# mobiusml/hqq

Measured on NVIDIA H100. Metric: llama3_8b_4bit_gs64_decode_tokens_per_s, higher is better.
Workload: dtype f16

## Files before the change

hqq_b200/csrc/linear_small.cu:

```cuda
#include <string.h>
#include <type_traits>

#include "linear_internal.cuh"

namespace hqq {


constexpr int kMaxProb = 4;

struct SKProb {
  const uint8_t* Wq;
  const void* scale;
  const void* zero;
  const void* bias;
  void* y;
  uint32_t* ytag;
  int N;
  int step;
  int tile0;
};

struct SKArgs {
  SKProb p[kMaxProb];
  int nprob;
  const void* x;
  int M, K;
  int Gk;
  int KB;
  int total_tiles;
  int xop;
  int yop;
  const void* x2;
  const void* xw;
  void* h_out;
  float eps;
  int tp, rank;
  uint32_t* peer_data[8];
  const uint32_t* red_data;
  const uint32_t* xtag;
  const uint32_t* x2tag;
  const int* step_ctr;
  int x_index, x_per_step;
};

#ifdef HQQ_EMU
#define HQQ_ST_RELAXED_SYS(p, v) (*reinterpret_cast<volatile uint32_t*>(p) = (v))
#else
#define HQQ_ST_RELAXED_SYS(p, v) asm volatile("st.relaxed.sys.global.u32 [%0], %1;" ::"l"(p), "r"(v) : "memory")
#endif

template <typename T> struct MT16;
template <> struct MT16<__half> {
  static constexpr uint32_t ONE2 = 0x3C003C00u;
  __device__ __forceinline__ static void mma(float (&d)[4], uint32_t a0, uint32_t a1, uint32_t a2, uint32_t a3, uint32_t b0, uint32_t b1) {
#ifndef HQQ_EMU
    asm volatile("mma.sync.aligned.m16n8k16.row.col.f32.f16.f16.f32 {%0,%1,%2,%3}, {%4,%5,%6,%7}, {%8,%9}, {%0,%1,%2,%3};"
                 : "+f"(d[0]), "+f"(d[1]), "+f"(d[2]), "+f"(d[3])
                 : "r"(a0), "r"(a1), "r"(a2), "r"(a3), "r"(b0), "r"(b1));
#else
    ::emu::mma_m16n8k16<__half>(d, a0, a1, a2, a3, b0, b1, false);
#endif
  }
  __device__ __forceinline__ static void mma0(float (&d)[4], uint32_t a0, uint32_t a1, uint32_t a2, uint32_t a3, uint32_t b0, uint32_t b1) {
#ifndef HQQ_EMU
    asm volatile("mma.sync.aligned.m16n8k16.row.col.f32.f16.f16.f32 {%0,%1,%2,%3}, {%4,%5,%6,%7}, {%8,%9}, {%10,%10,%10,%10};"
                 : "=f"(d[0]), "=f"(d[1]), "=f"(d[2]), "=f"(d[3])
                 : "r"(a0), "r"(a1), "r"(a2), "r"(a3), "r"(b0), "r"(b1), "f"(0.0f));
#else
    ::emu::mma_m16n8k16<__half>(d, a0, a1, a2, a3, b0, b1, true);
#endif
  }
  __device__ __forceinline__ static float ld(const void* p, long long i) { return __half2float(reinterpret_cast<const __half*>(p)[i]); }
  __device__ __forceinline__ static __half cvt(float v, const void* bias, int n) {
    __half o = __float2half_rn(v);
    if (bias) o = __hadd(o, reinterpret_cast<const __half*>(bias)[n]);
    return o;
  }
  __device__ __forceinline__ static void st(void* p, long long i, float v, const void* bias, int n) { reinterpret_cast<__half*>(p)[i] = cvt(v, bias, n); }
};
template <> struct MT16<__nv_bfloat16> {
  static constexpr uint32_t ONE2 = 0x3F803F80u;
  __device__ __forceinline__ static void mma(float (&d)[4], uint32_t a0, uint32_t a1, uint32_t a2, uint32_t a3, uint32_t b0, uint32_t b1) {
#ifndef HQQ_EMU
    asm volatile("mma.sync.aligned.m16n8k16.row.col.f32.bf16.bf16.f32 {%0,%1,%2,%3}, {%4,%5,%6,%7}, {%8,%9}, {%0,%1,%2,%3};"
                 : "+f"(d[0]), "+f"(d[1]), "+f"(d[2]), "+f"(d[3])
                 : "r"(a0), "r"(a1), "r"(a2), "r"(a3), "r"(b0), "r"(b1));
#else
    ::emu::mma_m16n8k16<__nv_bfloat16>(d, a0, a1, a2, a3, b0, b1, false);
#endif
  }
  __device__ __forceinline__ static void mma0(float (&d)[4], uint32_t a0, uint32_t a1, uint32_t a2, uint32_t a3, uint32_t b0, uint32_t b1) {
#ifndef HQQ_EMU
    asm volatile("mma.sync.aligned.m16n8k16.row.col.f32.bf16.bf16.f32 {%0,%1,%2,%3}, {%4,%5,%6,%7}, {%8,%9}, {%10,%10,%10,%10};"
                 : "=f"(d[0]), "=f"(d[1]), "=f"(d[2]), "=f"(d[3])
                 : "r"(a0), "r"(a1), "r"(a2), "r"(a3), "r"(b0), "r"(b1), "f"(0.0f));
#else
    ::emu::mma_m16n8k16<__nv_bfloat16>(d, a0, a1, a2, a3, b0, b1, true);
#endif
  }
  __device__ __forceinline__ static float ld(const void* p, long long i) { return __bfloat162float(reinterpret_cast<const __nv_bfloat16*>(p)[i]); }
  __device__ __forceinline__ static __nv_bfloat16 cvt(float v, const void* bias, int n) {
    __nv_bfloat16 o = __float2bfloat16_rn(v);
    if (bias) o = __hadd(o, reinterpret_cast<const __nv_bfloat16*>(bias)[n]);
    return o;
  }
  __device__ __forceinline__ static void st(void* p, long long i, float v, const void* bias, int n) { reinterpret_cast<__nv_bfloat16*>(p)[i] = cvt(v, bias, n); }
};

template <int LUT>
__device__ __forceinline__ uint32_t lop3(uint32_t a, uint32_t b, uint32_t c) {
#ifdef HQQ_EMU
  return ::emu::lop3(a, b, c, (uint32_t)LUT);
#else
  uint32_t r;
  asm("lop3.b32 %0, %1, %2, %3, %4;" : "=r"(r) : "r"(a), "r"(b), "r"(c), "n"(LUT));
  return r;
#endif
}
__device__ __forceinline__ uint32_t and_or(uint32_t a, uint32_t b, uint32_t c) { return lop3<0xEA>(a, b, c); }

template <typename T, int NBITS> struct Lanes;

template <int NBITS>
struct Lanes<__half, NBITS> {
  static constexpr uint32_t OR = 0x64006400u;
  uint32_t mask_a, mask_b;
  float invV_a, invV_b, offV_a, offV_b;
  __device__ __forceinline__ void init(int sh_a, int sh_b) {
    const uint32_t m = (1u << NBITS) - 1u;
    mask_a = (m << sh_a) * 0x00010001u;
    mask_b = (m << sh_b) * 0x00010001u;
    invV_a = exp2f(-(float)sh_a); invV_b = exp2f(-(float)sh_b);
    offV_a = 1024.0f * invV_a;    offV_b = 1024.0f * invV_b;
  }
  __device__ __forceinline__ void extract(uint32_t w, uint32_t& a0, uint32_t& a1, uint32_t& a2, uint32_t& a3) const {
    const uint32_t wp = prmt(w, 0u, 0x3120u);
    const uint32_t wh = wp >> 8;
    a0 = and_or(wp, mask_a, OR);
    a1 = and_or(wp, mask_b, OR);
    a2 = and_or(wh, mask_a, OR);
    a3 = and_or(wh, mask_b, OR);
  }
  __device__ __forceinline__ void extract_np(uint32_t w, uint32_t& a0, uint32_t& a1, uint32_t& a2, uint32_t& a3) const {
    const uint32_t wh = w >> 8;
    a0 = and_or(w, mask_a, OR);
    a1 = and_or(w, mask_b, OR);
    a2 = and_or(wh, mask_a, OR);
    a3 = and_or(wh, mask_b, OR);
  }
};

template <int NBITS>
struct Lanes<__nv_bfloat16, NBITS> {
  int sh_a, sh_b;
  float invV_a, invV_b, offV_a, offV_b;
  __device__ __forceinline__ void init(int sa, int sb) {
    sh_a = sa; sh_b = sb;
    invV_a = invV_b = 1.0f;
    offV_a = offV_b = 128.0f;
  }
  __device__ __forceinline__ void extract(uint32_t w, uint32_t& a0, uint32_t& a1, uint32_t& a2, uint32_t& a3) const {
    constexpr uint32_t M = ((1u << NBITS) - 1u) * 0x00010001u;
    const uint32_t wp = prmt(w, 0u, 0x3120u);
    a0 = and_or(wp >> sh_a, M, 0x43004300u);
    a1 = and_or(wp >> sh_b, M, 0x43004300u);
    a2 = and_or(wp >> (sh_a + 8), M, 0x43004300u);
    a3 = and_or(wp >> (sh_b + 8), M, 0x43004300u);
  }
  __device__ __forceinline__ void extract_np(uint32_t w, uint32_t& a0, uint32_t& a1, uint32_t& a2, uint32_t& a3) const {
    constexpr uint32_t M = ((1u << NBITS) - 1u) * 0x00010001u;
    a0 = and_or(w >> sh_a, M, 0x43004300u);
    a1 = and_or(w >> sh_b, M, 0x43004300u);
    a2 = and_or(w >> (sh_a + 8), M, 0x43004300u);
    a3 = and_or(w >> (sh_b + 8), M, 0x43004300u);
  }
};

template <>
struct Lanes<__half, 8> {
  static constexpr uint32_t HB = 0x64646464u;
  float invV_a, invV_b, offV_a, offV_b;
  __device__ __forceinline__ void init(int, int) { invV_a = invV_b = 1.0f; offV_a = offV_b = 1024.0f; }
  __device__ __forceinline__ void extract2(uint32_t wa, uint32_t wb, uint32_t& a0, uint32_t& a1, uint32_t& a2, uint32_t& a3) const {
    a0 = prmt(wa, HB, 0x4140u);
    a2 = prmt(wa, HB, 0x4342u);
    a1 = prmt(wb, HB, 0x4140u);
    a3 = prmt(wb, HB, 0x4342u);
  }
  __device__ __forceinline__ void extract2_np(uint32_t wa, uint32_t wb, uint32_t& a0, uint32_t& a1, uint32_t& a2, uint32_t& a3) const {
    a0 = prmt(wa, HB, 0x4240u);
    a2 = prmt(wa, HB, 0x4341u);
    a1 = prmt(wb, HB, 0x4240u);
    a3 = prmt(wb, HB, 0x4341u);
  }
};

__device__ __forceinline__ void cp_async16(void* smem, const void* g) {
#ifdef HQQ_EMU
  ::emu::cp_async(smem, g, 16);
#else
  const uint32_t s = (uint32_t)__cvta_generic_to_shared(smem);
  asm volatile("cp.async.cg.shared.global [%0], [%1], 16;" ::"r"(s), "l"(g) : "memory");
#endif
}
#ifdef HQQ_EMU
__device__ __forceinline__ void cp_async_commit() { ::emu::cp_async_commit(); }
template <int N> __device__ __forceinline__ void cp_async_wait() { ::emu::cp_async_wait(N); }
#else
__device__ __forceinline__ void cp_async_commit() { asm volatile("cp.async.commit_group;" ::: "memory"); }
template <int N>
__device__ __forceinline__ void cp_async_wait() { asm volatile("cp.async.wait_group %0;" ::"n"(N) : "memory"); }
#endif

template <typename T> __device__ __forceinline__ T from_f32_t(float v);
template <> __device__ __forceinline__ __half from_f32_t<__half>(float v) { return __float2half_rn(v); }
template <> __device__ __forceinline__ __nv_bfloat16 from_f32_t<__nv_bfloat16>(float v) { return __float2bfloat16_rn(v); }

template <typename T, int NBITS, int GS, int MT>
struct SKCfg {
  static constexpr int F = 8 / NBITS;
  static constexpr int P = 16 / F;
  static constexpr int MPG = GS / 16;
  static constexpr int GPB = 256 / GS;
  static constexpr int NWV = (F == 1) ? 8 : 4;
  static constexpr int ST = (F == 1) ? 2 : 4;
  static constexpr int W_BYTES = ST * NWV * 256 * 16;
  static constexpr int P_BYTES = 2 * 8 * MT * 128 * 4;
  static constexpr int SMEM = W_BYTES + P_BYTES;
  static constexpr int MIN_CTAS = (SMEM <= 110 * 1024 && MT <= 2) ? 2 : 1;
};

template <typename T, int NBITS, int GS, int MT>
__global__ void __launch_bounds__(256, SKCfg<T, NBITS, GS, MT>::MIN_CTAS) linear_small_kernel(const __grid_constant__ SKArgs a) {
  using C = SKCfg<T, NBITS, GS, MT>;
  constexpr int F = C::F, P = C::P, MPG = C::MPG, GPB = C::GPB, NWV = C::NWV, ST = C::ST;
  using MM = MT16<T>;
  extern __shared__ __align__(16) uint8_t smem[];
  uint4* wring = reinterpret_cast<uint4*>(smem);
  float* part_s = reinterpret_cast<float*>(smem + C::W_BYTES);

  const int tid = threadIdx.x, warp = tid >> 5, lane = tid & 31;
  const int r = lane >> 2, c = lane & 3;
  const int p = (F == 1) ? r : (r % P);
  const int fa = (F == 1) ? 0 : (r / P), fb = (F == 1) ? 0 : (F / 2 + r / P);
  Lanes<T, NBITS> lanes;
  lanes.init(8 - NBITS * (fa + 1), 8 - NBITS * (fb + 1));

  const int kb0 = a.KB * warp / 8, kb1 = a.KB * (warp + 1) / 8;
  const int upt = kb1 - kb0;
  const int n_tiles = (a.total_tiles - (int)blockIdx.x + (int)gridDim.x - 1) / (int)gridDim.x;
  if (n_tiles <= 0) return;

  struct Tile {
    const uint8_t* Wq; const T* scale; const T* zero; const T* bias; T* y;
    int N, step, tile0;
  };
  auto locate = [&](int gt, Tile& t) {
    int pi = 0;
#pragma unroll
    for (int i = 1; i < kMaxProb; ++i)
      if (i < a.nprob && gt >= a.p[i].tile0) pi = i;
    const uint8_t* Wq = a.p[0].Wq; const void* sc = a.p[0].scale; const void* ze = a.p[0].zero; const void* bi = a.p[0].bias;
    void* y = a.p[0].y; int N = a.p[0].N, step = a.p[0].step, tile0 = a.p[0].tile0;
#pragma unroll
    for (int i = 1; i < kMaxProb; ++i)
      if (pi == i) { Wq = a.p[i].Wq; sc = a.p[i].scale; ze = a.p[i].zero; bi = a.p[i].bias; y = a.p[i].y; N = a.p[i].N; step = a.p[i].step; tile0 = a.p[i].tile0; }
    t.Wq = Wq; t.scale = reinterpret_cast<const T*>(sc); t.zero = reinterpret_cast<const T*>(ze);
    t.bias = reinterpret_cast<const T*>(bi); t.y = reinterpret_cast<T*>(y); t.N = N; t.step = step; t.tile0 = tile0;
  };
  auto rows = [&](int gt, Tile& t, int& prow_a, int& prow_b) {
    locate(gt, t);
    prow_a = (gt - t.tile0) * P + p;
    prow_b = (F == 1) ? prow_a + 8 : prow_a;
  };

  int i_tile = 0, i_k = 0;
  const uint8_t *iw_a, *iw_b;
  auto issue_setup = [&]() {
    Tile t; int prow_a, prow_b;
    rows((int)blockIdx.x + i_tile * (int)gridDim.x, t, prow_a, prow_b);
    const long long ra = prow_a < t.step ? prow_a : 0, rb = prow_b < t.step ? prow_b : 0;
    iw_a = t.Wq + ra * a.K + (long long)kb0 * 256 + 16 * c;
    iw_b = t.Wq + rb * a.K + (long long)kb0 * 256 + 16 * c;
  };
  int to_issue = n_tiles * upt;
  if (to_issue > 0) issue_setup();
  int m_tile = 0, m_k = 0, m_left = n_tiles * upt;
  const T *ms_a = nullptr, *mz_a = nullptr, *ms_b = nullptr, *mz_b = nullptr;
  auto meta_setup = [&]() {
    const int gt = (int)blockIdx.x + m_tile * (int)gridDim.x;
    Tile t; int prow_a, prow_b;
    rows(gt, t, prow_a, prow_b);
    const long long na = prow_a < t.step ? fa * t.step + prow_a : 0, nb = prow_b < t.step ? fb * t.step + prow_b : 0;
    ms_a = t.scale + na * a.Gk + kb0 * GPB; mz_a = t.zero + na * a.Gk + kb0 * GPB;
    ms_b = t.scale + nb * a.Gk + kb0 * GPB; mz_b = t.zero + nb * a.Gk + kb0 * GPB;
  };
  if (m_left > 0) meta_setup();
  Vec<T, GPB> mv[4];
  auto meta_fetch = [&]() {
    if (m_left > 0) {
      mv[0] = *reinterpret_cast<const Vec<T, GPB>*>(ms_a); mv[1] = *reinterpret_cast<const Vec<T, GPB>*>(mz_a);
      mv[2] = *reinterpret_cast<const Vec<T, GPB>*>(ms_b); mv[3] = *reinterpret_cast<const Vec<T, GPB>*>(mz_b);
      --m_left;
      if (++m_k == upt) {
        m_k = 0; ++m_tile;
        if (m_left > 0) meta_setup();
      } else {
        ms_a += GPB; mz_a += GPB; ms_b += GPB; mz_b += GPB;
      }
    }
  };
  meta_fetch();
  auto issue = [&](int stage) {
    if (to_issue > 0) {
#pragma unroll
      for (int i = 0; i < 4; ++i) cp_async16(&wring[(stage * NWV + i) * 256 + tid], iw_a + i * 64);
      if (F == 1) {
#pragma unroll
        for (int i = 0; i < 4; ++i) cp_async16(&wring[(stage * NWV + 4 + i) * 256 + tid], iw_b + i * 64);
      }
      --to_issue;
      if (++i_k == upt) {
        i_k = 0; ++i_tile;
        if (to_issue > 0) issue_setup();
      } else {
        iw_a += 256; iw_b += 256;
      }
    }
    cp_async_commit();
  };
#pragma unroll
  for (int s = 0; s < ST - 1; ++s) issue(s);
  pdl_launch_dependents();
  pdl_wait();

  const T* xbase[MT];
#pragma unroll
  for (int mt = 0; mt < MT; ++mt) {
    const int m = min(mt * 8 + r, a.M - 1);
    xbase[mt] = reinterpret_cast<const T*>(a.x) + (long long)m * a.K + 16 * c;
  }
  uint4 xa[MT], xb[MT];
  auto load_x = [&](int kb, int us) {
#pragma unroll
    for (int mt = 0; mt < MT; ++mt) {
      const uint4* q = reinterpret_cast<const uint4*>(xbase[mt] + kb * 256 + us * 64);
      xa[mt] = __ldg(q);
      xb[mt] = __ldg(q + 1);
    }
  };
  if (upt > 0) load_x(kb0, 0);

  int stage = 0;
  for (int ti = 0; ti < n_tiles; ++ti) {
    float tot[MT][4];
#pragma unroll
    for (int mt = 0; mt < MT; ++mt)
#pragma unroll
      for (int i = 0; i < 4; ++i) tot[mt][i] = 0.0f;

    for (int ku = 0; ku < upt; ++ku) {
      {
        int is = stage + (ST - 1);
        if (is >= ST) is -= ST;
        issue(is);
      }
      cp_async_wait<ST - 1>();

      float sA[GPB], zA[GPB], sB[GPB], zB[GPB];
#pragma unroll
      for (int i = 0; i < GPB; ++i) { sA[i] = to_f32<T>(mv[0].v[i]); zA[i] = to_f32<T>(mv[1].v[i]); sB[i] = to_f32<T>(mv[2].v[i]); zB[i] = to_f32<T>(mv[3].v[i]); }
      meta_fetch();
      const int kb = kb0 + ku;
      const int kb_next = (ku + 1 == upt) ? kb0 : kb + 1;
      float Sg[MT][4], Xg[MT][4];
#pragma unroll
      for (int us = 0; us < 4; ++us) {
        uint4 ya[MT], yb[MT];
#pragma unroll
        for (int mt = 0; mt < MT; ++mt) { ya[mt] = xa[mt]; yb[mt] = xb[mt]; }
        if (us < 3) load_x(kb, us + 1); else load_x(kb_next, 0);
        const uint4 va = wring[(stage * NWV + us) * 256 + tid];
        uint4 vb = va;
        if (F == 1) vb = wring[(stage * NWV + 4 + us) * 256 + tid];
        const uint32_t wa[4] = {va.x, va.y, va.z, va.w};
        const uint32_t wb[4] = {vb.x, vb.y, vb.z, vb.w};
#pragma unroll
        for (int j = 0; j < 4; ++j) {
          uint32_t a0, a1, a2, a3;
          if constexpr (F == 1) lanes.extract2(wa[j], wb[j], a0, a1, a2, a3);
          else lanes.extract(wa[j], a0, a1, a2, a3);
          const bool first = ((us * 4 + j) % MPG) == 0;
#pragma unroll
          for (int mt = 0; mt < MT; ++mt) {
            const uint32_t b0 = (j == 0) ? ya[mt].x : (j == 1) ? ya[mt].z : (j == 2) ? yb[mt].x : yb[mt].z;
            const uint32_t b1 = (j == 0) ? ya[mt].y : (j == 1) ? ya[mt].w : (j == 2) ? yb[mt].y : yb[mt].w;
            if (first) {
              MM::mma0(Sg[mt], a0, a1, a2, a3, b0, b1);
              MM::mma0(Xg[mt], MM::ONE2, MM::ONE2, MM::ONE2, MM::ONE2, b0, b1);
            } else {
              MM::mma(Sg[mt], a0, a1, a2, a3, b0, b1);
              MM::mma(Xg[mt], MM::ONE2, MM::ONE2, MM::ONE2, MM::ONE2, b0, b1);
            }
          }
          if (((us * 4 + j + 1) % MPG) == 0) {
            const int gi = (us * 4 + j) / MPG;
            const float ka = sA[gi] * lanes.invV_a, la = -sA[gi] * (lanes.offV_a + zA[gi]);
            const float kb2 = sB[gi] * lanes.invV_b, lb = -sB[gi] * (lanes.offV_b + zB[gi]);
#pragma unroll
            for (int mt = 0; mt < MT; ++mt) {
              tot[mt][0] = fmaf(ka, Sg[mt][0], fmaf(la, Xg[mt][0], tot[mt][0]));
              tot[mt][1] = fmaf(ka, Sg[mt][1], fmaf(la, Xg[mt][1], tot[mt][1]));
              tot[mt][2] = fmaf(kb2, Sg[mt][2], fmaf(lb, Xg[mt][0], tot[mt][2]));
              tot[mt][3] = fmaf(kb2, Sg[mt][3], fmaf(lb, Xg[mt][1], tot[mt][3]));
            }
          }
        }
      }
      if (++stage == ST) stage = 0;
    }

    float* buf = part_s + (ti & 1) * (8 * MT * 128);
#pragma unroll
    for (int mt = 0; mt < MT; ++mt)
      *reinterpret_cast<float4*>(buf + (warp * MT + mt) * 128 + lane * 4) = make_float4(tot[mt][0], tot[mt][1], tot[mt][2], tot[mt][3]);
    __syncthreads();
    if (warp == (ti & 7)) {
      Tile t; int prow_a, prow_b;
      rows((int)blockIdx.x + ti * (int)gridDim.x, t, prow_a, prow_b);
      const bool ok_a = prow_a < t.step, ok_b = prow_b < t.step;
      const int n_a = fa * t.step + prow_a, n_b = fb * t.step + prow_b;
#pragma unroll
      for (int mt = 0; mt < MT; ++mt) {
        float4 acc = make_float4(0.f, 0.f, 0.f, 0.f);
#pragma unroll
        for (int w = 0; w < 8; ++w) {
          const float4 v = *reinterpret_cast<const float4*>(buf + (w * MT + mt) * 128 + lane * 4);
          acc.x += v.x; acc.y += v.y; acc.z += v.z; acc.w += v.w;
        }
        const int m0 = mt * 8 + 2 * c;
        if (m0 < a.M) {
          if (ok_a) MM::st(t.y, (long long)m0 * t.N + n_a, acc.x, t.bias, n_a);
          if (ok_b) MM::st(t.y, (long long)m0 * t.N + n_b, acc.z, t.bias, n_b);
        }
        if (m0 + 1 < a.M) {
          if (ok_a) MM::st(t.y, (long long)(m0 + 1) * t.N + n_a, acc.y, t.bias, n_a);
          if (ok_b) MM::st(t.y, (long long)(m0 + 1) * t.N + n_b, acc.w, t.bias, n_b);
        }
      }
    }
  }
  cp_async_wait<0>();
}

template <typename T, int NBITS, int GS, int ST, int MR = 0>
struct D1Cfg {
  static constexpr int F = 8 / NBITS, P = 16 / F, MPG = GS / 16, GPB = 256 / GS;
  static constexpr int NWV = (F == 1) ? 8 : 4;
  static constexpr int W_BYTES = ST * NWV * 256 * 16;
  static constexpr int M_BYTES = (MR & 1) ? ST * 8 * 4 * 8 * 16 : 0;
  static constexpr int P_BYTES = 2 * 8 * 16 * 4;
  static int smem(int K) { return W_BYTES + M_BYTES + P_BYTES + K * 2 + (K / GS) * 4; }
};

template <typename T, int NBITS, int GS, int ST, int MC, int MR = 0>
__global__ void __launch_bounds__(256, MC) linear_decode1_kernel(const __grid_constant__ SKArgs a) {
  using C = D1Cfg<T, NBITS, GS, ST, MR>;
  constexpr int F = C::F, P = C::P, MPG = C::MPG, GPB = C::GPB, NWV = C::NWV;
  using MM = MT16<T>;
  extern __shared__ __align__(16) uint8_t smem[];
  uint4* wring = reinterpret_cast<uint4*>(smem);
  uint4* mring = reinterpret_cast<uint4*>(smem + C::W_BYTES);
  float* part_s = reinterpret_cast<float*>(smem + C::W_BYTES + C::M_BYTES);
  T* xs = reinterpret_cast<T*>(smem + C::W_BYTES + C::M_BYTES + C::P_BYTES);
  float* xsum = reinterpret_cast<float*>(smem + C::W_BYTES + C::M_BYTES + C::P_BYTES + a.K * 2);

  const int tid = threadIdx.x, warp = tid >> 5, lane = tid & 31;
  const int r = lane >> 2, c = lane & 3;
  const int p = (F == 1) ? r : (r % P);
  const int fa = (F == 1) ? 0 : (r / P), fb = (F == 1) ? 0 : (F / 2 + r / P);
  Lanes<T, NBITS> lanes;
  lanes.init(8 - NBITS * (fa + 1), 8 - NBITS * (fb + 1));

  const int kb0 = a.KB * warp / 8, kb1 = a.KB * (warp + 1) / 8;
  const int upt = kb1 - kb0;
  const int n_tiles = (a.total_tiles - (int)blockIdx.x + (int)gridDim.x - 1) / (int)gridDim.x;
  if (n_tiles <= 0) return;

  struct Tile { const uint8_t* Wq; const T* scale; const T* zero; const T* bias; T* y; uint32_t* ytag; int N, step, tile0; };
  auto pick = [&](int pi, Tile& t) {
    const uint8_t* Wq = a.p[0].Wq; const void* sc = a.p[0].scale; const void* ze = a.p[0].zero; const void* bi = a.p[0].bias;
    void* y = a.p[0].y; uint32_t* yt = a.p[0].ytag; int N = a.p[0].N, step = a.p[0].step, tile0 = a.p[0].tile0;
#pragma unroll
    for (int i = 1; i < kMaxProb; ++i)
      if (pi == i) { Wq = a.p[i].Wq; sc = a.p[i].scale; ze = a.p[i].zero; bi = a.p[i].bias; y = a.p[i].y; yt = a.p[i].ytag; N = a.p[i].N; step = a.p[i].step; tile0 = a.p[i].tile0; }
    t.Wq = Wq; t.scale = reinterpret_cast<const T*>(sc); t.zero = reinterpret_cast<const T*>(ze);
    t.bias = reinterpret_cast<const T*>(bi); t.y = reinterpret_cast<T*>(y); t.ytag = yt; t.N = N; t.step = step; t.tile0 = tile0;
  };
  auto locate = [&](int gt, Tile& t) {
    int pi = 0;
#pragma unroll
    for (int i = 1; i < kMaxProb; ++i)
      if (i < a.nprob && gt >= a.p[i].tile0) pi = i;
    pick(pi, t);
  };
  constexpr int PH = (P >= 2) ? P / 2 : 1;
  const bool paired = (F > 1) && a.yop == 1;
  auto rows = [&](int gt, Tile& t, int& prow_a, int& prow_b) {
    if (paired) {
      pick(p >= PH ? 1 : 0, t);
      prow_a = prow_b = gt * PH + (p % PH);
    } else {
      locate(gt, t);
      prow_a = (gt - t.tile0) * P + p;
      prow_b = (F == 1) ? prow_a + 8 : prow_a;
    }
  };

  int i_tile = 0, i_k = 0;
  const uint8_t *iw_a, *iw_b;
  const T* im = nullptr;
  auto issue_setup = [&]() {
    Tile t; int prow_a, prow_b;
    rows((int)blockIdx.x + i_tile * (int)gridDim.x, t, prow_a, prow_b);
    const long long ra = prow_a < t.step ? prow_a : 0, rb = prow_b < t.step ? prow_b : 0;
    iw_a = t.Wq + ra * a.K + (long long)kb0 * 256 + 16 * c;
    iw_b = t.Wq + rb * a.K + (long long)kb0 * 256 + 16 * c;
    if constexpr ((MR & 1) != 0) {
      const long long na = prow_a < t.step ? fa * t.step + prow_a : 0, nb = prow_b < t.step ? fb * t.step + prow_b : 0;
      im = ((c & 1) ? t.zero : t.scale) + ((c & 2) ? nb : na) * a.Gk + kb0 * GPB;
    }
  };
  int to_issue = n_tiles * upt;
  if (to_issue > 0) issue_setup();
  int m_tile = 0, m_k = 0, m_left = (MR & 1) ? 0 : n_tiles * upt;
  const T *ms_a = nullptr, *mz_a = nullptr, *ms_b = nullptr, *mz_b = nullptr;
  auto meta_setup = [&]() {
    const int gt = (int)blockIdx.x + m_tile * (int)gridDim.x;
    Tile t; int prow_a, prow_b;
    rows(gt, t, prow_a, prow_b);
    const long long na = prow_a < t.step ? fa * t.step + prow_a : 0, nb = prow_b < t.step ? fb * t.step + prow_b : 0;
    ms_a = t.scale + na * a.Gk + kb0 * GPB; mz_a = t.zero + na * a.Gk + kb0 * GPB;
    ms_b = t.scale + nb * a.Gk + kb0 * GPB; mz_b = t.zero + nb * a.Gk + kb0 * GPB;
  };
  if (m_left > 0) meta_setup();
  Vec<T, GPB> mv[4];
  auto meta_fetch = [&]() {
    if (m_left > 0) {
      mv[0] = *reinterpret_cast<const Vec<T, GPB>*>(ms_a); mv[1] = *reinterpret_cast<const Vec<T, GPB>*>(mz_a);
      mv[2] = *reinterpret_cast<const Vec<T, GPB>*>(ms_b); mv[3] = *reinterpret_cast<const Vec<T, GPB>*>(mz_b);
      --m_left;
      if (++m_k == upt) {
        m_k = 0; ++m_tile;
        if (m_left > 0) meta_setup();
      } else {
        ms_a += GPB; mz_a += GPB; ms_b += GPB; mz_b += GPB;
      }
    }
  };
  meta_fetch();
  auto issue = [&](int stage) {
    if (to_issue > 0) {
#pragma unroll
      for (int i = 0; i < 4; ++i) cp_async16(&wring[(stage * NWV + i) * 256 + tid], iw_a + i * 64);
      if (F == 1) {
#pragma unroll
        for (int i = 0; i < 4; ++i) cp_async16(&wring[(stage * NWV + 4 + i) * 256 + tid], iw_b + i * 64);
      }
      if constexpr ((MR & 1) != 0)
        cp_async16(&mring[((stage * 8 + warp) * 4 + c) * 8 + r], reinterpret_cast<const void*>(reinterpret_cast<uintptr_t>(im) & ~uintptr_t(15)));
      --to_issue;
      if (++i_k == upt) {
        i_k = 0; ++i_tile;
        if (to_issue > 0) issue_setup();
      } else {
        iw_a += 256; iw_b += 256;
        if constexpr ((MR & 1) != 0) im += GPB;
      }
    }
    cp_async_commit();
  };
#pragma unroll
  for (int s = 0; s < ST - 1; ++s) issue(s);
  pdl_launch_dependents();
  pdl_wait();
  uint32_t send_tag = 0, send_par = 0;
  if (a.step_ctr) {
    const uint32_t ex = (uint32_t)(*reinterpret_cast<volatile const int*>(a.step_ctr)) * (uint32_t)a.x_per_step + (uint32_t)a.x_index;
    send_tag = ex & 0xFFFFu;
    send_par = ex & 1u;
  }

  {
    const T* x = reinterpret_cast<const T*>(a.x);
    const T* x2 = reinterpret_cast<const T*>(a.x2);
    const int k_lo = kb0 * 256, k_hi = kb1 * 256;
    float inv = 1.0f;
    const uint32_t* red = nullptr;
    const uint32_t rtag = send_tag;
    if (a.xop == 1 && a.red_data) red = a.red_data + (size_t)send_par * a.tp * a.K;
    auto poll8 = [&](const uint32_t* src, Vec<T, 8>& out) {
      uint4 w0, w1;
      bool ok;
      do {
#ifdef HQQ_EMU
        memcpy(&w0, src, 16); memcpy(&w1, src + 4, 16);
#else
        asm volatile("ld.relaxed.sys.global.v4.u32 {%0,%1,%2,%3}, [%4];" : "=r"(w0.x), "=r"(w0.y), "=r"(w0.z), "=r"(w0.w) : "l"(src) : "memory");
        asm volatile("ld.relaxed.sys.global.v4.u32 {%0,%1,%2,%3}, [%4];" : "=r"(w1.x), "=r"(w1.y), "=r"(w1.z), "=r"(w1.w) : "l"(src + 4) : "memory");
#endif
        ok = ((w0.x >> 16) == rtag) & ((w0.y >> 16) == rtag) & ((w0.z >> 16) == rtag) & ((w0.w >> 16) == rtag) &
             ((w1.x >> 16) == rtag) & ((w1.y >> 16) == rtag) & ((w1.z >> 16) == rtag) & ((w1.w >> 16) == rtag);
      } while (!ok);
      const uint32_t ws[8] = {w0.x, w0.y, w0.z, w0.w, w1.x, w1.y, w1.z, w1.w};
#pragma unroll
      for (int j = 0; j < 8; ++j) {
        const unsigned short hb = (unsigned short)(ws[j] & 0xFFFFu);
        out.v[j] = *reinterpret_cast<const T*>(&hb);
      }
    };
    auto delta8 = [&](int k8, Vec<T, 8>& d) -> bool {
      if (red) {
        float acc[8];
#pragma unroll
        for (int j = 0; j < 8; ++j) acc[j] = 0.0f;
        for (int rr = 0; rr < a.tp; ++rr) {
          Vec<T, 8> p8;
          poll8(red + (size_t)rr * a.K + k8, p8);
#pragma unroll
          for (int j = 0; j < 8; ++j) acc[j] += to_f32<T>(p8.v[j]);
        }
#pragma unroll
        for (int j = 0; j < 8; ++j) d.v[j] = from_f32_t<T>(acc[j]);
        return true;
      }
      if (x2) { d = *reinterpret_cast<const Vec<T, 8>*>(x2 + k8); return true; }
      return false;
    };
    auto put_permuted = [&](int k8, const Vec<T, 8>& v) {
      Vec<T, 8> w;
      w.v[0] = v.v[0]; w.v[1] = v.v[2]; w.v[2] = v.v[1]; w.v[3] = v.v[3];
      w.v[4] = v.v[4]; w.v[5] = v.v[6]; w.v[6] = v.v[5]; w.v[7] = v.v[7];
      *reinterpret_cast<Vec<T, 8>*>(xs + k8) = w;
    };
    if (a.xop == 1) {
      const T* xw = reinterpret_cast<const T*>(a.xw);
      T* hout = reinterpret_cast<T*>(a.h_out);
      const int kg0 = k_lo + lane * 8;
      Vec<T, 8> g0, g1;
      if (kg0 < k_hi) g0 = *reinterpret_cast<const Vec<T, 8>*>(xw + kg0);
      if (kg0 + 256 < k_hi) g1 = *reinterpret_cast<const Vec<T, 8>*>(xw + kg0 + 256);
      float ss = 0.0f;
      for (int ka = tid * 8; ka < a.K; ka += 2 * 256 * 8) {
        const int kb = ka + 256 * 8;
        const bool has_b = kb < a.K;
        Vec<T, 8> va = *reinterpret_cast<const Vec<T, 8>*>(x + ka), vb, da, db;
        if (has_b) vb = *reinterpret_cast<const Vec<T, 8>*>(x + kb);
        const bool add_a = delta8(ka, da);
        const bool add_b = has_b && delta8(kb, db);
        if (add_a) {
#pragma unroll
          for (int j = 0; j < 8; ++j) va.v[j] = from_f32_t<T>(to_f32<T>(va.v[j]) + to_f32<T>(da.v[j]));
        }
        if (add_b) {
#pragma unroll
          for (int j = 0; j < 8; ++j) vb.v[j] = from_f32_t<T>(to_f32<T>(vb.v[j]) + to_f32<T>(db.v[j]));
        }
        *reinterpret_cast<Vec<T, 8>*>(xs + ka) = va;
        if (has_b) *reinterpret_cast<Vec<T, 8>*>(xs + kb) = vb;
        if (hout && blockIdx.x == 0) {
          *reinterpret_cast<Vec<T, 8>*>(hout + ka) = va;
          if (has_b) *reinterpret_cast<Vec<T, 8>*>(hout + kb) = vb;
        }
#pragma unroll
        for (int j = 0; j < 8; ++j) { const float f = to_f32<T>(va.v[j]); ss += f * f; }
        if (has_b) {
#pragma unroll
          for (int j = 0; j < 8; ++j) { const float f = to_f32<T>(vb.v[j]); ss += f * f; }
        }
      }
#pragma unroll
      for (int o = 16; o > 0; o >>= 1) ss += __shfl_xor_sync(0xffffffffu, ss, o);
      if (lane == 0) part_s[warp] = ss;
      __syncthreads();
      float tot = 0.0f;
#pragma unroll
      for (int w = 0; w < 8; ++w) tot += part_s[w];
      inv = rsqrtf(tot / (float)a.K + a.eps);
      __syncthreads();
      int i = 0;
      for (int k8 = kg0; k8 < k_hi; k8 += 256, ++i) {
        Vec<T, 8> v = *reinterpret_cast<const Vec<T, 8>*>(xs + k8);
        const Vec<T, 8> g = (i == 0) ? g0 : (i == 1) ? g1 : *reinterpret_cast<const Vec<T, 8>*>(xw + k8);
#pragma unroll
        for (int j = 0; j < 8; ++j) v.v[j] = from_f32_t<T>(to_f32<T>(from_f32_t<T>(to_f32<T>(v.v[j]) * inv)) * to_f32<T>(g.v[j]));
        put_permuted(k8, v);
      }
    } else {
      for (int k8 = k_lo + lane * 8; k8 < k_hi; k8 += 256) {
        Vec<T, 8> v;
        if (a.xop == 2 && a.xtag) poll8(a.xtag + (size_t)send_par * a.K + k8, v);
        else v = *reinterpret_cast<const Vec<T, 8>*>(x + k8);
        if (a.xop == 2) {
          Vec<T, 8> u;
          if (a.x2tag) poll8(a.x2tag + (size_t)send_par * a.K + k8, u);
          else u = *reinterpret_cast<const Vec<T, 8>*>(x2 + k8);
#pragma unroll
          for (int j = 0; j < 8; ++j) {
            const float f = to_f32<T>(v.v[j]);
            v.v[j] = from_f32_t<T>(to_f32<T>(from_f32_t<T>(f / (1.0f + __expf(-f)))) * to_f32<T>(u.v[j]));
          }
        }
        put_permuted(k8, v);
      }
    }
    __syncwarp();
    for (int g = k_lo / GS + lane; g < k_hi / GS; g += 32) {
      float acc = 0.0f;
#pragma unroll 4
      for (int i = 0; i < GS; i += 8) {
        const Vec<T, 8> v = *reinterpret_cast<const Vec<T, 8>*>(xs + g * GS + i);
#pragma unroll
        for (int j = 0; j < 8; ++j) acc += to_f32<T>(v.v[j]);
      }
      xsum[g] = acc;
    }
    __syncwarp();
  }

  int stage = 0;
  for (int ti = 0; ti < n_tiles; ++ti) {
    float tot_a = 0.0f, tot_b = 0.0f;
    for (int ku = 0; ku < upt; ++ku) {
      {
        int is = stage + (ST - 1);
        if (is >= ST) is -= ST;
        issue(is);
      }
      cp_async_wait<ST - 1>();
      const int kb = kb0 + ku;
      float sA[GPB], zA[GPB], sB[GPB], zB[GPB];
      if constexpr ((MR & 1) != 0) {
        __syncwarp();
        const char* mr = reinterpret_cast<const char*>(mring + ((stage * 8 + warp) * 4) * 8) + r * 16 + ((kb * GPB * 2) & 15);
#pragma unroll
        for (int v = 0; v < 4; ++v) mv[v] = *reinterpret_cast<const Vec<T, GPB>*>(mr + v * 128);
      }
#pragma unroll
      for (int i = 0; i < GPB; ++i) { sA[i] = to_f32<T>(mv[0].v[i]); zA[i] = to_f32<T>(mv[1].v[i]); sB[i] = to_f32<T>(mv[2].v[i]); zB[i] = to_f32<T>(mv[3].v[i]); }
      if constexpr ((MR & 1) == 0) meta_fetch();
      const T* xk = xs + kb * 256 + 16 * c;
      float Sg[4];
#pragma unroll
      for (int us = 0; us < 4; ++us) {
        const uint4 xa = *reinterpret_cast<const uint4*>(xk + us * 64);
        const uint4 xb = *reinterpret_cast<const uint4*>(xk + us * 64 + 8);
        const uint4 va = wring[(stage * NWV + us) * 256 + tid];
        uint4 vb = va;
        if (F == 1) vb = wring[(stage * NWV + 4 + us) * 256 + tid];
        const uint32_t wa[4] = {va.x, va.y, va.z, va.w};
        const uint32_t wb[4] = {vb.x, vb.y, vb.z, vb.w};
#pragma unroll
        for (int j = 0; j < 4; ++j) {
          uint32_t a0, a1, a2, a3;
          if constexpr (F == 1) lanes.extract2_np(wa[j], wb[j], a0, a1, a2, a3);
          else lanes.extract_np(wa[j], a0, a1, a2, a3);
          const uint32_t b0 = (j == 0) ? xa.x : (j == 1) ? xa.z : (j == 2) ? xb.x : xb.z;
          const uint32_t b1 = (j == 0) ? xa.y : (j == 1) ? xa.w : (j == 2) ? xb.y : xb.w;
          if (((us * 4 + j) % MPG) == 0) MM::mma0(Sg, a0, a1, a2, a3, b0, b1);
          else MM::mma(Sg, a0, a1, a2, a3, b0, b1);
          if (((us * 4 + j + 1) % MPG) == 0) {
            const int gi = (us * 4 + j) / MPG;
            const float X = xsum[kb * GPB + gi];
            tot_a = fmaf(sA[gi] * lanes.invV_a, Sg[0], fmaf(-sA[gi] * (lanes.offV_a + zA[gi]), X, tot_a));
            tot_b = fmaf(sB[gi] * lanes.invV_b, Sg[2], fmaf(-sB[gi] * (lanes.offV_b + zB[gi]), X, tot_b));
          }
        }
      }
      if (++stage == ST) stage = 0;
    }
    float* buf = part_s + (ti & 1) * 128;
    if (c == 0) { buf[warp * 16 + r] = tot_a; buf[warp * 16 + 8 + r] = tot_b; }
    __syncthreads();
    if (warp == (ti & 7) && lane < 16) {
      const int gt = (int)blockIdx.x + ti * (int)gridDim.x;
      const int rr = lane & 7, hi = lane >> 3;
      const int pp = (F == 1) ? rr : (rr % P);
      const int ff = (F == 1) ? 0 : (hi ? F / 2 + rr / P : rr / P);
      if (paired) {
        Tile tg, tu; pick(0, tg); pick(1, tu);
        const int prow = gt * PH + pp;
        if (pp < PH && prow < tg.step) {
          float ag = 0.0f, au = 0.0f;
#pragma unroll
          for (int w = 0; w < 8; ++w) { ag += buf[w * 16 + lane]; au += buf[w * 16 + lane + PH]; }
          const int n = ff * tg.step + prow;
          const float f = to_f32<T>(MM::cvt(ag, tg.bias, n));
          const float u = to_f32<T>(MM::cvt(au, tu.bias, n));
          tg.y[n] = from_f32_t<T>(to_f32<T>(from_f32_t<T>(f / (1.0f + __expf(-f)))) * u);
        }
        continue;
      }
      Tile t; locate(gt, t);
      const int prow = (gt - t.tile0) * P + pp + ((F == 1 && hi) ? 8 : 0);
      if (prow < t.step) {
        float acc = 0.0f;
#pragma unroll
        for (int w = 0; w < 8; ++w) acc += buf[w * 16 + lane];
        const int n = ff * t.step + prow;
        MM::st(t.y, n, acc, t.bias, n);
        if (a.peer_data[0] || t.ytag) {
          const T pv = from_f32_t<T>(acc);
          const uint32_t word = (send_tag << 16) | (uint32_t)(*reinterpret_cast<const unsigned short*>(&pv));
          if (a.peer_data[0]) {
            const size_t off = ((size_t)send_par * a.tp + a.rank) * t.N + n;
#pragma unroll
            for (int dst = 0; dst < 8; ++dst)
              if (dst < a.tp) HQQ_ST_RELAXED_SYS(a.peer_data[dst] + off, word);
          }
          if (t.ytag) HQQ_ST_RELAXED_SYS(t.ytag + (size_t)send_par * t.N + n, word);
        }
      }
    }
  }
  cp_async_wait<0>();
}

template <typename T, int NBITS, int GS, int MT>
static int launch_sk(SKArgs& a, cudaStream_t st) {
  using C = SKCfg<T, NBITS, GS, MT>;
  int rc = reserve_smem<linear_small_kernel<T, NBITS, GS, MT>>(C::SMEM);
  if (rc) return rc;
  static int per_sm[kMaxDevices] = {};
  int& occ = per_sm[current_device()];
  if (!occ) {
    int n = 0;
    cudaError_t e = cudaOccupancyMaxActiveBlocksPerMultiprocessor(&n, linear_small_kernel<T, NBITS, GS, MT>, 256, C::SMEM);
    HQQ_REQUIRE(e == cudaSuccess && n > 0, HQQ_E_CUDA, "hqq_b200_linear_fwd: occupancy query failed: %s", cudaGetErrorString(e));
    occ = n > 2 ? 2 : n;
  }
  const int max_grid = sm_count() * occ;
  return launch_pdl("hqq_b200_linear_fwd/small", linear_small_kernel<T, NBITS, GS, MT>, dim3((unsigned)(a.total_tiles < max_grid ? a.total_tiles : max_grid)),
                    dim3(256), C::SMEM, st, a);
}

template <typename T, int NBITS, int GS, int ST, int MC, int MR = 0>
static int launch_d1(SKArgs& a, cudaStream_t st) {
  const int smem = D1Cfg<T, NBITS, GS, ST, MR>::smem(a.K);
  int rc = reserve_smem<linear_decode1_kernel<T, NBITS, GS, ST, MC, MR>>(smem);
  if (rc) return rc;
  int per_sm = MC;
  while (per_sm > 1 && (smem + 1024) * per_sm > 227 * 1024) --per_sm;
  const int max_grid = sm_count() * per_sm;
  return launch_pdl("hqq_b200_linear_fwd/decode1", linear_decode1_kernel<T, NBITS, GS, ST, MC, MR>,
                    dim3((unsigned)(a.total_tiles < max_grid ? a.total_tiles : max_grid)), dim3(256), smem, st, a);
}

bool small_xop_ok(int64_t M, int64_t K) { return M == 1 && K <= 16384; }

template <typename T, int NBITS, int GS>
static int sk_mt(SKArgs& a, cudaStream_t st) {
  if (small_xop_ok(a.M, a.K)) {
    if constexpr (NBITS == 8) {
      return launch_d1<T, NBITS, GS, 2, 2>(a, st);
    } else {
      if constexpr (GS == 64) {
        if (a.K % 512 == 0) {
          bool ok = true;
          for (int i = 0; i < a.nprob; ++i) ok = ok && aligned(a.p[i].scale, 16) && aligned(a.p[i].zero, 16);
          if (ok) return launch_d1<T, NBITS, GS, 4, 2, 1>(a, st);
        }
      }
      return launch_d1<T, NBITS, GS, 4, 2>(a, st);
    }
  }
  if (a.M <= 8) return launch_sk<T, NBITS, GS, 1>(a, st);
  if (a.M <= 16) return launch_sk<T, NBITS, GS, 2>(a, st);
  return launch_sk<T, NBITS, GS, 4>(a, st);
}

template <typename T, int NBITS>
static int sk_gs(SKArgs& a, int gs, cudaStream_t st) {
  switch (gs) {
    case 64: return sk_mt<T, NBITS, 64>(a, st);
    case 128: return sk_mt<T, NBITS, 128>(a, st);
  }
  return HQQ_E_UNSUPPORTED;
}

template <typename T>
static int sk_bits(SKArgs& a, int gs, int nbits, cudaStream_t st) {
  switch (nbits) {
    case 8:
      if constexpr (std::is_same<T, __half>::value) return sk_gs<T, 8>(a, gs, st);
      else return HQQ_E_UNSUPPORTED;
    case 4: return sk_gs<T, 4>(a, gs, st);
    case 2: return sk_gs<T, 2>(a, gs, st);
    case 1: return sk_gs<T, 1>(a, gs, st);
  }
  return HQQ_E_UNSUPPORTED;
}

bool small_route_ok(int64_t M, int64_t N, int64_t K, int gs, int nbits, int axis, int dtype) {
  if (axis != 1) return false;
  if (dtype != HQQ_F16 && dtype != HQQ_BF16) return false;
  if (!(nbits == 8 || nbits == 4 || nbits == 2 || nbits == 1)) return false;
  if (nbits == 8 && dtype == HQQ_BF16) return false;
  if (!(gs == 64 || gs == 128)) return false;
  if (M < 1 || M > 32) return false;
  if (K % 256 != 0 || K % gs != 0) return false;
  if (N % (8 / nbits) != 0) return false;
  if (N > (1 << 28) || K > (1 << 28)) return false;
  return true;
}

size_t small_workspace_bytes(int64_t) { return 0; }

int linear_small_multi(const void* x, int nprob, const void* const* Wq, const void* const* scale, const void* const* zero,
                       const void* const* bias, void* const* y, const int64_t* N, int64_t M, int64_t K, int gs, int nbits, int dtype,
                       void* ws, size_t ws_bytes, cudaStream_t st, int xop, const void* x2, const void* xw, void* h_out, float eps,
                       const TpExchange* tpx) {
  HQQ_REQUIRE(nprob >= 1 && nprob <= kMaxProb, HQQ_E_INVALID, "hqq_b200_linear_fwd_multi: 1..%d matrices per launch (got %d)", kMaxProb, nprob);
  HQQ_REQUIRE(aligned(x, 16), HQQ_E_INVALID, "hqq_b200_linear_fwd: x must be 16-byte aligned");
  (void)ws; (void)ws_bytes;
  const int F = 8 / nbits, P = 16 / F;
  SKArgs a;
  a.nprob = nprob; a.x = x; a.M = (int)M; a.K = (int)K; a.Gk = (int)(K / gs); a.KB = (int)(K / 256);
  const int yop = xop >> 4;
  xop &= 15;
  a.xop = xop; a.yop = yop; a.x2 = x2; a.xw = xw; a.h_out = h_out; a.eps = eps;
  if (yop) {
    HQQ_REQUIRE(yop == 1, HQQ_E_INVALID, "hqq_b200_decode_linear_fwd: unknown epilogue %d", yop);
    HQQ_REQUIRE(nprob == 2 && N[0] == N[1], HQQ_E_INVALID, "hqq_b200_decode_linear_fwd: the silu*mul epilogue pairs exactly two matrices of equal N");
    if (!(small_xop_ok(M, K) && nbits < 8) || (tpx && (tpx->peer_data || tpx->y_tagged))) {
      set_error("hqq_b200_decode_linear_fwd: the silu*mul epilogue needs the M == 1 kernel, nbits < 8 and plain outputs");
      return HQQ_E_UNSUPPORTED;
    }
  }
  a.tp = 1; a.rank = 0; a.red_data = nullptr; a.xtag = nullptr; a.x2tag = nullptr; a.step_ctr = nullptr; a.x_index = 0; a.x_per_step = 1;
  for (int i = 0; i < 8; ++i) a.peer_data[i] = nullptr;
  if (tpx && !tpx->step_ctr) tpx = nullptr;
  if (tpx) {
    HQQ_REQUIRE(small_xop_ok(M, K) && nprob >= 1, HQQ_E_UNSUPPORTED, "hqq_b200_decode_linear_fwd_desc: needs the M == 1 kernel");
    HQQ_REQUIRE(tpx->tp >= 1 && tpx->tp <= 8 && tpx->rank >= 0 && tpx->rank < tpx->tp && tpx->step_ctr && tpx->x_per_step > 0, HQQ_E_INVALID,
                "hqq_b200_decode_linear_fwd_desc: bad tp/rank/step counter");
    a.tp = tpx->tp; a.rank = tpx->rank; a.step_ctr = tpx->step_ctr; a.x_index = tpx->x_index; a.x_per_step = tpx->x_per_step;
    if (tpx->peer_data) {
      HQQ_REQUIRE(nprob == 1, HQQ_E_INVALID, "hqq_b200_decode_linear_fwd_desc: the scatter side takes exactly one matrix");
      for (int i = 0; i < tpx->tp; ++i) a.peer_data[i] = reinterpret_cast<uint32_t*>(tpx->peer_data[i]);
    }
    if (tpx->red_data) {
      HQQ_REQUIRE(xop == 1, HQQ_E_INVALID, "hqq_b200_decode_linear_fwd_desc: a reduced delta needs x_op 1");
      a.red_data = reinterpret_cast<const uint32_t*>(tpx->red_data);
    }
    if (tpx->x_tagged || tpx->x2_tagged) {
      HQQ_REQUIRE(xop == 2 && tpx->x_tagged && tpx->x2_tagged, HQQ_E_INVALID, "hqq_b200_decode_linear_fwd_desc: tagged activations need x_op 2 and both operands");
      a.xtag = reinterpret_cast<const uint32_t*>(tpx->x_tagged); a.x2tag = reinterpret_cast<const uint32_t*>(tpx->x2_tagged);
    }
  }
  int tiles = 0;
  for (int i = 0; i < kMaxProb; ++i) {
    const int j = i < nprob ? i : 0;
    HQQ_REQUIRE(Wq[j] && scale[j] && zero[j] && y[j], HQQ_E_INVALID, "hqq_b200_linear_fwd: null pointer");
    HQQ_REQUIRE(aligned(Wq[j], 16) && aligned(scale[j], 8) && aligned(zero[j], 8), HQQ_E_INVALID,
                "hqq_b200_linear_fwd: W_q must be 16-byte and scale/zero 8-byte aligned");
    a.p[i].Wq = (const uint8_t*)Wq[j]; a.p[i].scale = scale[j]; a.p[i].zero = zero[j]; a.p[i].bias = bias ? bias[j] : nullptr;
    a.p[i].y = y[j]; a.p[i].ytag = (tpx && tpx->y_tagged) ? reinterpret_cast<uint32_t*>(tpx->y_tagged[j]) : nullptr; a.p[i].N = (int)N[j]; a.p[i].step = (int)(N[j] / F); a.p[i].tile0 = tiles;
    if (i < nprob) tiles += (int)cdiv(a.p[i].step, P);
  }
  a.total_tiles = yop ? (int)cdiv(a.p[0].step, P / 2) : tiles;
  if (dtype == HQQ_F16) return sk_bits<__half>(a, gs, nbits, st);
  return sk_bits<__nv_bfloat16>(a, gs, nbits, st);
}

}
```

Baseline: 429.9.

## Use one CTA per SM with 3-stage pipeline for small decode GEMVs

For M=1 decode layers with few tiles (at most four per SM), launches the decode kernel with a 3-stage cp.async ring and forces one CTA per SM by padding dynamic shared memory past half the SM capacity. Scale/zero metadata is kept as packed half vectors and converted to float only where each group is consumed, which lowers register pressure. The goal is to spread few tiles evenly across SMs rather than doubling up CTAs on some SMs, and to free registers. The cost is a shallower prefetch pipeline and an extra device attribute query.

```diff
diff --git a/hqq_b200/csrc/linear_small.cu b/hqq_b200/csrc/linear_small.cu
--- a/hqq_b200/csrc/linear_small.cu
+++ b/hqq_b200/csrc/linear_small.cu
@@ -739,15 +739,15 @@
       }
       cp_async_wait<ST - 1>();
       const int kb = kb0 + ku;
-      float sA[GPB], zA[GPB], sB[GPB], zB[GPB];
       if constexpr ((MR & 1) != 0) {
         __syncwarp();
         const char* mr = reinterpret_cast<const char*>(mring + ((stage * 8 + warp) * 4) * 8) + r * 16 + ((kb * GPB * 2) & 15);
 #pragma unroll
         for (int v = 0; v < 4; ++v) mv[v] = *reinterpret_cast<const Vec<T, GPB>*>(mr + v * 128);
       }
-#pragma unroll
-      for (int i = 0; i < GPB; ++i) { sA[i] = to_f32<T>(mv[0].v[i]); zA[i] = to_f32<T>(mv[1].v[i]); sB[i] = to_f32<T>(mv[2].v[i]); zB[i] = to_f32<T>(mv[3].v[i]); }
+      Vec<T, GPB> mu[4];
+#pragma unroll
+      for (int v = 0; v < 4; ++v) mu[v] = mv[v];
       if constexpr ((MR & 1) == 0) meta_fetch();
       const T* xk = xs + kb * 256 + 16 * c;
       float Sg[4];
@@ -772,8 +772,9 @@
           if (((us * 4 + j + 1) % MPG) == 0) {
             const int gi = (us * 4 + j) / MPG;
             const float X = xsum[kb * GPB + gi];
-            tot_a = fmaf(sA[gi] * lanes.invV_a, Sg[0], fmaf(-sA[gi] * (lanes.offV_a + zA[gi]), X, tot_a));
-            tot_b = fmaf(sB[gi] * lanes.invV_b, Sg[2], fmaf(-sB[gi] * (lanes.offV_b + zB[gi]), X, tot_b));
+            const float sA = to_f32<T>(mu[0].v[gi]), zA = to_f32<T>(mu[1].v[gi]), sB = to_f32<T>(mu[2].v[gi]), zB = to_f32<T>(mu[3].v[gi]);
+            tot_a = fmaf(sA * lanes.invV_a, Sg[0], fmaf(-sA * (lanes.offV_a + zA), X, tot_a));
+            tot_b = fmaf(sB * lanes.invV_b, Sg[2], fmaf(-sB * (lanes.offV_b + zB), X, tot_b));
           }
         }
       }
@@ -844,12 +845,26 @@
                     dim3(256), C::SMEM, st, a);
 }
 
+static int half_sm_smem() {
+  static int cached[kMaxDevices] = {};
+  int& r = cached[current_device()];
+  if (!r) {
+    const int dev = current_device();
+    int per_sm = 0, reserved = 0;
+    if (cudaDeviceGetAttribute(&per_sm, cudaDevAttrMaxSharedMemoryPerMultiprocessor, dev) != cudaSuccess || per_sm <= 0) per_sm = 228 * 1024;
+    if (cudaDeviceGetAttribute(&reserved, cudaDevAttrReservedSharedMemoryPerBlock, dev) != cudaSuccess || reserved < 0) reserved = 1024;
+    r = per_sm / 2 - reserved;
+  }
+  return r;
+}
+
 template <typename T, int NBITS, int GS, int ST, int MC, int MR = 0>
-static int launch_d1(SKArgs& a, cudaStream_t st) {
-  const int smem = D1Cfg<T, NBITS, GS, ST, MR>::smem(a.K);
+static int launch_d1(SKArgs& a, cudaStream_t st, int ctas_per_sm = MC) {
+  int smem = D1Cfg<T, NBITS, GS, ST, MR>::smem(a.K);
+  if (ctas_per_sm == 1 && smem <= half_sm_smem()) smem = half_sm_smem() + 16;
   int rc = reserve_smem<linear_decode1_kernel<T, NBITS, GS, ST, MC, MR>>(smem);
   if (rc) return rc;
-  int per_sm = MC;
+  int per_sm = ctas_per_sm < MC ? ctas_per_sm : MC;
   while (per_sm > 1 && (smem + 1024) * per_sm > 227 * 1024) --per_sm;
   const int max_grid = sm_count() * per_sm;
   return launch_pdl("hqq_b200_linear_fwd/decode1", linear_decode1_kernel<T, NBITS, GS, ST, MC, MR>,
@@ -864,14 +879,15 @@
     if constexpr (NBITS == 8) {
       return launch_d1<T, NBITS, GS, 2, 2>(a, st);
     } else {
+      const bool few = a.total_tiles <= 4 * sm_count();
       if constexpr (GS == 64) {
         if (a.K % 512 == 0) {
           bool ok = true;
           for (int i = 0; i < a.nprob; ++i) ok = ok && aligned(a.p[i].scale, 16) && aligned(a.p[i].zero, 16);
-          if (ok) return launch_d1<T, NBITS, GS, 4, 2, 1>(a, st);
-        }
-      }
-      return launch_d1<T, NBITS, GS, 4, 2>(a, st);
+          if (ok) return few ? launch_d1<T, NBITS, GS, 3, 2, 1>(a, st, 1) : launch_d1<T, NBITS, GS, 4, 2, 1>(a, st);
+        }
+      }
+      return few ? launch_d1<T, NBITS, GS, 3, 2>(a, st, 1) : launch_d1<T, NBITS, GS, 4, 2>(a, st);
     }
   }
   if (a.M <= 8) return launch_sk<T, NBITS, GS, 1>(a, st);
```

After: 435.2 (median of 6 runs). 1.01x the previous value.
